# ruc-aimc-lab/GeoFormer

Hardware: AMD Instinct MI355X
Metric: image-pairs/sec (640x640) (higher is better)
Workload: dtype f16

## Files before the change

### geoformer_amd/csrc/k9_encoder_fused.hip

```cpp
#include <math.h>

#include <type_traits>

#include "gf_common.h"
#include "k9_args.h"

#ifndef K9P_TRACE
#define K9P_TRACE 0
#endif
#ifndef K9P_ABLATE
#define K9P_ABLATE 0
#endif
#if K9P_TRACE
__device__ long long k9p_trace[1024 * 8 * 24];
#define K9P_T(slot) do { if (lane == 0 && blockIdx.x < 1024) k9p_trace[(blockIdx.x * 8 + wave) * 24 + (slot)] = (long long)__builtin_amdgcn_s_memtime(); } while (0)
extern "C" int gf_debug_k9p_trace(long long* out) {
    return (int)hipMemcpyFromSymbol(out, HIP_SYMBOL(k9p_trace), sizeof(long long) * 1024 * 8 * 24);
}
#else
#define K9P_T(slot)
#endif

namespace {

constexpr int C = 256, D = 32, NH = 8;
constexpr int TM = 128;
constexpr int FRAG = 1024, BLK = 16 * FRAG;
constexpr int X_OFF = 0;
constexpr int W_OFF = 65536;
constexpr int E_OFF = W_OFF + 3 * BLK;
constexpr int VEC_OFF = E_OFF + 32768;
constexpr int KS_OFF = VEC_OFF + 4 * C * 4;
constexpr int ST_OFF = KS_OFF + 512;
constexpr int LDS_BYTES = ST_OFF + 8 * 64 * 8;
constexpr int NB_Q = 8, NB_M = 8, NB_SLICE = 12, NB_KV = 16;

using EncArgs = GfEncArgs;

template <typename T>
__device__ __forceinline__ typename Mma32<T>::Frag pack8(float a0, float a1, float a2, float a3, float a4, float a5, float a6,
                                                          float a7) {
    typedef T t2 __attribute__((ext_vector_type(2)));
    typedef float f2 __attribute__((ext_vector_type(2)));
    const t2 p0 = __builtin_convertvector(f2{a0, a1}, t2), p1 = __builtin_convertvector(f2{a2, a3}, t2);
    const t2 p2 = __builtin_convertvector(f2{a4, a5}, t2), p3 = __builtin_convertvector(f2{a6, a7}, t2);
    return typename Mma32<T>::Frag{p0[0], p0[1], p1[0], p1[1], p2[0], p2[1], p3[0], p3[1]};
}
template <typename T>
__device__ __forceinline__ typename Mma32<T>::Frag pack_step(const v16f& a, int s) {
    return s == 0 ? pack8<T>(a[0], a[1], a[2], a[3], a[4], a[5], a[6], a[7])
                  : pack8<T>(a[8], a[9], a[10], a[11], a[12], a[13], a[14], a[15]);
}
template <typename F>
__device__ __forceinline__ F relu_packed(const F& f) {
    typedef short v8s __attribute__((ext_vector_type(8)));
    const v8s x = __builtin_bit_cast(v8s, f);
    return __builtin_bit_cast(F, x & ~(x >> 15));
}
__device__ __forceinline__ float phi(float x) {
    return fmaxf(x, 0.f) + __builtin_amdgcn_fmed3f(__builtin_amdgcn_exp2f(x * 1.44269504088896341f), 0.f, 1.f);
}
__device__ __forceinline__ v16f zero16() { return v16f{0.f, 0.f, 0.f, 0.f, 0.f, 0.f, 0.f, 0.f, 0.f, 0.f, 0.f, 0.f, 0.f, 0.f, 0.f, 0.f}; }
__device__ __forceinline__ int fresh_lane() {
    int l;
    asm volatile("v_mbcnt_lo_u32_b32 %0, -1, 0\n\tv_mbcnt_hi_u32_b32 %0, -1, %0" : "=v"(l));
    return l;
}
__device__ __forceinline__ float half_sum(float x) {
    const gf_v2u sw = __builtin_amdgcn_permlane32_swap(__float_as_uint(x), __float_as_uint(x), false, false);
    return __uint_as_float(sw.x) + __uint_as_float(sw.y);
}
__device__ __forceinline__ float dot8(const v8h& a, const v8h& b, float c) {
    typedef _Float16 h2 __attribute__((ext_vector_type(2)));
#pragma unroll
    for (int i = 0; i < 4; ++i) c = __builtin_amdgcn_fdot2(h2{a[2 * i], a[2 * i + 1]}, h2{b[2 * i], b[2 * i + 1]}, c, false);
    return c;
}
__device__ __forceinline__ float dot8(const v8b& a, const v8b& b, float c) {
    typedef __bf16 b2 __attribute__((ext_vector_type(2)));
#pragma unroll
    for (int i = 0; i < 4; ++i) c = __builtin_amdgcn_fdot2_f32_bf16(b2{a[2 * i], a[2 * i + 1]}, b2{b[2 * i], b[2 * i + 1]}, c, false);
    return c;
}

template <typename T>
struct PMma {
    static __device__ __forceinline__ void mma(const typename Mma32<T>::Frag& a, const typename Mma32<T>::Frag& b, v16f& c) {
#if K9P_ABLATE == 4
        asm volatile("" : "+v"(c) : "v"(a), "v"(b));
#else
        Mma32<T>::mma(a, b, c);
#endif
    }
};

struct Ring {
    __amdgpu_buffer_rsrc_t rs;
    __amdgpu_buffer_rsrc_t rs2;
    char* smem;
    int voff;
    int wave;
    int rbase;
    int blk, nblk;
};
__device__ __forceinline__ Ring ring_make(const void* wstream, char* smem, int wave, int lane, int nblk, const void* wstream2, int nblk2) {
    return Ring{__builtin_amdgcn_make_buffer_rsrc(const_cast<void*>(wstream), 0, nblk * BLK, 0x00020000),
                __builtin_amdgcn_make_buffer_rsrc(const_cast<void*>(wstream2 ? wstream2 : wstream), 0, wstream2 ? nblk2 * BLK : 0, 0x00020000),
                smem, lane * 16 + wave * 2 * FRAG, wave, W_OFF + (wave & 1) * 8 * FRAG + lane * 16, 0, nblk};
}
__device__ __forceinline__ void dma_piece(const Ring& g, int slot, int b, int i) {
#if K9P_ABLATE == 1
    if (b >= 3) return;
#endif
    const bool second = b >= g.nblk;
    __builtin_amdgcn_raw_ptr_buffer_load_lds(second ? g.rs2 : g.rs,
                                             (__attribute__((address_space(3))) void*)(g.smem + W_OFF + slot * BLK + (g.wave * 2 + i) * FRAG), 16,
                                             g.voff, (second ? b - g.nblk : b) * BLK + i * FRAG, 0, 0);
}
template <int VM>
__device__ __forceinline__ void turn() {
    asm volatile("s_waitcnt vmcnt(%0) lgkmcnt(0)" ::"n"(VM) : "memory");
#if K9P_ABLATE != 2
    __builtin_amdgcn_s_barrier();
#endif
}
__device__ __forceinline__ void xbar() {
    asm volatile("s_waitcnt lgkmcnt(0)" ::: "memory");
    __builtin_amdgcn_s_barrier();
}
template <typename Frag>
__device__ __forceinline__ Frag lds_frag(const char* p) { return *reinterpret_cast<const Frag*>(p); }
template <typename Frag>
__device__ __forceinline__ Frag ring_frag(const char* p) {
#if K9P_ABLATE == 3
    Frag f; asm volatile("" : "=v"(f)); return f;
#else
    return *reinterpret_cast<const Frag*>(p);
#endif
}

#define K9_GAP(DMA, READS, VALU)                                            \
    __builtin_amdgcn_sched_group_barrier(0x008, 1, 0);                      \
    if (DMA) __builtin_amdgcn_sched_group_barrier(0x010, 1, 0);             \
    if (READS) __builtin_amdgcn_sched_group_barrier(0x100, READS, 0);       \
    if (VALU) __builtin_amdgcn_sched_group_barrier(0x002, VALU, 0);
template <int NX0, int NX4, int VM, int NV0 = 0, int NV4 = 0, typename Frag, typename MF, typename H0, typename H4>
__device__ __forceinline__ void pblock(Ring& g, Frag (&F)[8], int slot, MF mma, H0 h0, H4 h4) {
    const char* pc = g.smem + g.rbase + slot * BLK;
    mma(0);
    F[6] = ring_frag<Frag>(pc + 6 * FRAG);
    h0();
    mma(1);
    F[7] = ring_frag<Frag>(pc + 7 * FRAG);
    mma(2);
    mma(3);
    K9_GAP(false, 1 + NX0, NV0) K9_GAP(false, 1, NV0) K9_GAP(false, 0, NV0) K9_GAP(false, 0, NV0)
    __builtin_amdgcn_sched_barrier(0);
    turn<VM>();
    const char* p = g.smem + g.rbase + ((slot + 1) % 3) * BLK;
    mma(4);
    dma_piece(g, slot, g.blk + 3, 0);
    F[0] = ring_frag<Frag>(p);
    F[1] = ring_frag<Frag>(p + FRAG);
    h4();
    mma(5);
    dma_piece(g, slot, g.blk + 3, 1);
    F[2] = ring_frag<Frag>(p + 2 * FRAG);
    F[3] = ring_frag<Frag>(p + 3 * FRAG);
    mma(6);
    F[4] = ring_frag<Frag>(p + 4 * FRAG);
    mma(7);
    F[5] = ring_frag<Frag>(p + 5 * FRAG);
    K9_GAP(true, 2 + NX4, NV4) K9_GAP(true, 2, NV4) K9_GAP(false, 1, NV4) K9_GAP(false, 1, NV4)
    __builtin_amdgcn_sched_barrier(0);
    ++g.blk;
}
#undef K9_GAP
__device__ __forceinline__ void ring_start(const Ring& g) {
#pragma unroll
    for (int b = 0; b < 3; ++b) {
        dma_piece(g, b, b, 0);
        dma_piece(g, b, b, 1);
    }
    __builtin_amdgcn_sched_barrier(0);
}
template <typename Frag>
__device__ __forceinline__ void load_block0(const Ring& g, Frag (&f)[8]) {
    const char* p = g.smem + g.rbase;
#pragma unroll
    for (int i = 0; i < 6; ++i) f[i] = ring_frag<Frag>(p + i * FRAG);
}

template <typename T>
__device__ __forceinline__ void tile_dma(const T* base, long ld, int rows_total, int row0, int nrows, char* smem, int off, int wave, int lane,
                                         int waves) {
    const __amdgpu_buffer_rsrc_t rs = __builtin_amdgcn_make_buffer_rsrc(const_cast<T*>(base), 0, 0x7FFFFFFF, 0x00020000);
    const int planes_pieces = nrows / 8;
    const int total = 4 * planes_pieces, per = total / waves;
#pragma unroll
    for (int i = 0; i < 8; ++i) {
        if (i < per) {
            const int q = wave * per + i, kc = q / planes_pieces, rp = q - kc * planes_pieces;
            const int row = rp * 8 + (lane >> 3), c = (lane & 7) ^ ((row >> 1) & 7);
            const int r = min(row0 + row, rows_total - 1);
            __builtin_amdgcn_raw_ptr_buffer_load_lds(rs, (__attribute__((address_space(3))) void*)(smem + off + kc * (nrows * 128) + rp * 1024), 16,
                                                     (int)(r * ld * 2) + kc * 128 + c * 16, 0, 0, 0);
        }
    }
}

template <typename T>
__device__ __forceinline__ void kv_tail(Ring& ring, typename Mma32<T>::Frag (&F)[8], char* smem, unsigned valid,
                                        float* dst, int wave, int lane, int tid, int slot0);

template <typename T, int ACT, bool ATTN>
__global__ __launch_bounds__(512) void enc_layer(EncArgs a) {
    using Mm = Mma32<T>;
    using Frag = typename Mm::Frag;
    extern __shared__ __attribute__((aligned(16))) char smem[];
    const int tid = threadIdx.x, lane = tid & 63, wave = __builtin_amdgcn_readfirstlane(tid >> 6), h2 = lane >> 5, lr = lane & 31;
    const int w = wave & 1, grp = wave >> 1;
    const int n = blockIdx.x / a.tiles, tile = blockIdx.x - n * a.tiles;
    const int t0 = tile * TM;
    const T* xg = (const T*)a.x + (size_t)n * a.L * a.ldx;
    constexpr int NBLK = (ATTN ? NB_Q : 0) + NB_M + 4 * NB_SLICE;
    float* vec = reinterpret_cast<float*>(smem + VEC_OFF);
    const bool tail = ATTN && a.wstream_tail != nullptr && n >= a.tail_first;
    K9P_T(0);
    Ring ring = ring_make(a.wstream, smem, wave, lane, NBLK, tail ? a.wstream_tail : nullptr, NB_KV);
    const int mytok = t0 + grp * 32 + lr;
    const int myrow = grp * 32 + lr;
    const float lnv0 = a.ln[tid], lnv1 = a.ln[512 + tid];
    unsigned char qm = 1;
    if (a.q_mask != nullptr) qm = a.q_mask[(size_t)n * a.L + min(mytok, a.L - 1)];
    float kvv[2][8], ksv = 0.f;
    if constexpr (ATTN) {
        const float* kvf = a.kvfinal + (size_t)n * (C * D + C);
#pragma unroll
        for (int p = 0; p < 2; ++p) {
            const int sl = p * 512 + tid, ln = sl & 63, hs = sl >> 6, hh = hs >> 1, s = hs & 1;
            const float* src = kvf + (size_t)(hh * D + 16 * s + 4 * (ln >> 5)) * D + (ln & 31);
#pragma unroll
            for (int j = 0; j < 8; ++j) kvv[p][j] = src[((j >> 2) * 8 + (j & 3)) * D];
        }
        {
            const int tq = tid & 255, j = tq & 7, hx = (tq >> 3) & 1, sx = (tq >> 4) & 1, hh = tq >> 5;
            ksv = kvf[C * D + hh * D + 16 * sx + 8 * (j >> 2) + 4 * hx + (j & 3)];
        }
    }
    __builtin_amdgcn_sched_barrier(0);
    tile_dma<T>(xg, a.ldx, a.L, t0, TM, smem, X_OFF, wave, lane, 8);
    dma_piece(ring, 0, 0, 0);
    dma_piece(ring, 0, 0, 1);
    __builtin_amdgcn_sched_barrier(0);
    K9P_T(13);
    vec[tid] = lnv0;
    vec[512 + tid] = lnv1;
    const float qmul = qm != 0 ? 1.f : 0.f;
    if constexpr (ATTN) {
        const float inv_s = 1.0f / (float)a.S;
#pragma unroll
        for (int p = 0; p < 2; ++p) {
            const int sl = p * 512 + tid, ln = sl & 63, hs = sl >> 6;
            *reinterpret_cast<Frag*>(smem + E_OFF + hs * FRAG + ln * 16) =
                pack8<T>(kvv[p][0] * inv_s, kvv[p][1] * inv_s, kvv[p][2] * inv_s, kvv[p][3] * inv_s, kvv[p][4] * inv_s, kvv[p][5] * inv_s,
                         kvv[p][6] * inv_s, kvv[p][7] * inv_s);
        }
        reinterpret_cast<T*>(smem + KS_OFF)[tid & 255] = gf_from_float<T>(ksv * inv_s);
    }
    Frag ma[16];
    if constexpr (!ATTN) {
        const T* mg = (const T*)a.msg + (size_t)n * a.L * a.ldm;
#pragma unroll
        for (int half = 0; half < 2; ++half) {
            tile_dma<T>(mg, a.ldm, a.L, t0 + half * 64, 64, smem, E_OFF, wave, lane, 8);
            asm volatile("s_waitcnt vmcnt(0)" ::: "memory");
            __builtin_amdgcn_s_barrier();
            if ((grp >> 1) == half) {
                const int row = (grp & 1) * 32 + lr;
#pragma unroll
                for (int t = 0; t < 8; ++t)
#pragma unroll
                    for (int s = 0; s < 2; ++s) {
                        const int c0 = 32 * t + 16 * s + 4 * h2, ch = c0 >> 3;
                        const char* p0 = smem + E_OFF + (ch >> 3) * 8192 + gf_lds_off(row, ch & 7) + (c0 & 7) * 2;
                        const char* p1 = smem + E_OFF + ((ch + 1) >> 3) * 8192 + gf_lds_off(row, (ch + 1) & 7) + (c0 & 7) * 2;
                        typedef short v4s __attribute__((ext_vector_type(4)));
                        typedef short v8s __attribute__((ext_vector_type(8)));
                        const v4s lo = *reinterpret_cast<const v4s*>(p0), hi = *reinterpret_cast<const v4s*>(p1);
                        const v8s both = __builtin_shufflevector(lo, hi, 0, 1, 2, 3, 4, 5, 6, 7);
                        ma[2 * t + s] = __builtin_bit_cast(Frag, both);
                    }
            }
            xbar();
        }
    }
    K9P_T(14);
    asm volatile("s_waitcnt vmcnt(0) lgkmcnt(0)" ::: "memory");
    K9P_T(15);
    __builtin_amdgcn_s_barrier();
    dma_piece(ring, 1, 1, 0);
    dma_piece(ring, 1, 1, 1);
    dma_piece(ring, 2, 2, 0);
    dma_piece(ring, 2, 2, 1);
    __builtin_amdgcn_sched_barrier(0);

    K9P_T(1);
    Frag F[8];
    load_block0(ring, F);
    auto xfrag = [&](int ks) { return lds_frag<Frag>(smem + X_OFF + (ks >> 2) * 16384 + gf_lds_off(myrow, 2 * (ks & 3) + h2)); };
    char* const ex = smem + E_OFF + grp * 8192 + lane * 16;
    auto ex_put = [&](int i, const Frag& f) { *reinterpret_cast<Frag*>(ex + (4 * w + i) * FRAG) = f; };
    auto ex_get = [&](int s) { return lds_frag<Frag>(ex + s * FRAG); };
    int slot = 0;

    Frag kvf[4][2];
    v16f qacc[2];
    v16f num;
    float den = 0.f;
    Frag p0, p1, msg0, msg1;
    const float eps_s = ATTN ? a.attn_eps / (float)a.S : 0.f;
    auto att_a0 = [&](int t) {
        const int hh = 4 * w + t;
        const Frag ks0 = lds_frag<Frag>(smem + KS_OFF + ((hh * 2 + 0) * 2 + h2) * 16);
        const v16f& qh = qacc[t & 1];
        p0 = pack8<T>(phi(qh[0]), phi(qh[1]), phi(qh[2]), phi(qh[3]), phi(qh[4]), phi(qh[5]), phi(qh[6]), phi(qh[7]));
        den = dot8(p0, ks0, 0.f);
    };
    auto att_a1 = [&](int t) {
        const int hh = 4 * w + t;
        const Frag ks1 = lds_frag<Frag>(smem + KS_OFF + ((hh * 2 + 1) * 2 + h2) * 16);
        const v16f& qh = qacc[t & 1];
        p1 = pack8<T>(phi(qh[8]), phi(qh[9]), phi(qh[10]), phi(qh[11]), phi(qh[12]), phi(qh[13]), phi(qh[14]), phi(qh[15]));
        den = dot8(p1, ks1, den);
        num = zero16();
        Mm::mma(kvf[t][0], p0, num);
        Mm::mma(kvf[t][1], p1, num);
    };
    auto att_b0 = [&] {
        const float z = __builtin_amdgcn_rcpf(half_sum(den) + eps_s) * qmul;
#pragma unroll
        for (int r = 0; r < 16; ++r) num[r] *= z;
        msg0 = pack_step<T>(num, 0);
        msg1 = pack_step<T>(num, 1);
    };
    auto att_put = [&](int t) {
        *reinterpret_cast<Frag*>(ex + (4 * w + 2 * (t & 1)) * FRAG) = msg0;
        *reinterpret_cast<Frag*>(ex + (4 * w + 2 * (t & 1) + 1) * FRAG) = msg1;
    };
    auto att_get = [&](int t) {
        ma[2 * t] = ex_get(2 * (t & 1));
        ma[2 * t + 1] = ex_get(2 * (t & 1) + 1);
        ma[8 + 2 * t] = ex_get(4 + 2 * (t & 1));
        ma[9 + 2 * t] = ex_get(5 + 2 * (t & 1));
    };
    if constexpr (ATTN) {
#pragma unroll
// ... 170 lines not shown
        hn[1] = zero16();
        auto w1xn = [&](int j) { PMma<T>::mma(F[j], X[j >> 1], hn[j & 1]); };
#pragma unroll
        for (int b = 0; b < 4; ++b) {
            if (b < 3) pblock<2, 2, 2>(ring, F, slot, w1xn, [&] { xh0(b); }, [&] { xh4(b); });
            else pblock<2, 1, 2>(ring, F, slot, w1xn, [&] { xh0(b); }, [&] { H[0] = ex_get(0); });
            slot = (slot + 1) % 3;
        }
#pragma unroll
        for (int b = 0; b < 4; ++b) {
            pblock<1, 1, 2>(ring, F, slot, [&](int j) { PMma<T>::mma(F[j], H[j >> 2], o[j & 3]); }, [&] { H[1] = ex_get(2 * b + 1); },
                            [&] { if (b < 3) H[0] = ex_get(2 * b + 2); });
            slot = (slot + 1) % 3;
        }
#pragma unroll
        for (int b = 0; b < 4; ++b) {
            auto mm = [&](int j) { PMma<T>::mma(F[j], ma[4 * b + (j >> 1)], hn[j & 1]); };
            if (b < 3) pblock<0, 0, 2>(ring, F, slot, mm, [] {}, [] {});
            else pblock<0, 2, 2>(ring, F, slot, mm, [] {}, [&] { X[0] = xfrag(0); X[1] = xfrag(1); });
            slot = (slot + 1) % 3;
        }
        hd[0] = hn[0];
        hd[1] = hn[1];
        act_put();
    }
    K9P_T(8);
    {
        xbar();
        int slot = STAGE_SLOT;
        H[0] = ex_get(0);
#pragma unroll
        for (int b = 0; b < 4; ++b) {
            pblock<1, 1, 2>(ring, F, slot, [&](int j) { PMma<T>::mma(F[j], H[j >> 2], o[j & 3]); }, [&] { H[1] = ex_get(2 * b + 1); },
                            [&] { if (b < 3) H[0] = ex_get(2 * b + 2); });
            slot = (slot + 1) % 3;
        }
    }
    K9P_T(10);

    float mean2, rstd2;
    {
        float s2 = 0.f, q2 = 0.f;
#pragma unroll
        for (int t = 0; t < 4; ++t) stats_add(o[t], s2, q2);
        s2 = half_sum(s2);
        q2 = half_sum(q2);
        stats_put(s2, q2);
        xbar();
        stats_finish(s2, q2, a.eps2, mean2, rstd2);
    }
    const float nmr2 = -mean2 * rstd2;
    K9P_T(11);
    const bool keep = a.flag == nullptr || __builtin_amdgcn_readfirstlane(a.flag[((size_t)n * a.L + t0) / a.flag_rows]) != 0;
    {
        typedef T v4t __attribute__((ext_vector_type(4)));
        if (keep) {
            int xs[8];
#pragma unroll
            for (int k = 0; k < 8; ++k) xs[k] = X_OFF + w * 32768 + gf_lds_off(myrow, k) + h2 * 8;
            struct FinOps { v4t x[4]; LnOps ln[2]; };
            auto fin_ops = [&](int t) {
                FinOps fo;
#pragma unroll
                for (int g = 0; g < 4; ++g) fo.x[g] = *reinterpret_cast<const v4t*>(smem + xs[4 * (t & 1) + g] + (t >> 1) * 16384);
                fo.ln[0] = ln_ops(vec + 2 * C, vec + 3 * C, 4 * w + t, 0);
                fo.ln[1] = ln_ops(vec + 2 * C, vec + 3 * C, 4 * w + t, 1);
                return fo;
            };
            FinOps fo[2];
            fo[0] = fin_ops(0);
#pragma unroll
            for (int t = 0; t < 4; ++t) {
                if (t < 3) fo[(t + 1) & 1] = fin_ops(t + 1);
                const FinOps& p = fo[t & 1];
#pragma unroll
                for (int g = 0; g < 4; ++g) {
                    const v4f y = ln_apply(o[t], g, p.ln[g >> 1].ga[g & 1], p.ln[g >> 1].be[g & 1], nmr2, rstd2);
                    v4t ov;
                    ov[0] = gf_from_float<T>(gf_to_float(p.x[g][0]) + y.x);
                    ov[1] = gf_from_float<T>(gf_to_float(p.x[g][1]) + y.y);
                    ov[2] = gf_from_float<T>(gf_to_float(p.x[g][2]) + y.z);
                    ov[3] = gf_from_float<T>(gf_to_float(p.x[g][3]) + y.w);
                    *reinterpret_cast<v4t*>(smem + xs[4 * (t & 1) + g] + (t >> 1) * 16384) = ov;
                }
            }
            __builtin_amdgcn_fence(__ATOMIC_RELEASE, "wavefront");
            __builtin_amdgcn_wave_barrier();
            __builtin_amdgcn_fence(__ATOMIC_ACQUIRE, "wavefront");
        }
        K9P_T(17);
        T* og = (T*)a.out + (size_t)n * a.L * a.ldo;
        const __amdgpu_buffer_rsrc_t ors = __builtin_amdgcn_make_buffer_rsrc(og, 0, (int)min((long)a.L * a.ldo * 2, 0x7FFFFFFFL), 0x00020000);
        const int c16 = lane & 15, rsel = lane >> 4;
        v4u rows[8];
#pragma unroll
        for (int it = 0; it < 8; ++it)
            rows[it] = *reinterpret_cast<const v4u*>(smem + X_OFF + (2 * w + (c16 >> 3)) * 16384 + gf_lds_off(grp * 32 + 4 * it + rsel, c16 & 7));
#pragma unroll
        for (int it = 0; it < 8; ++it) {
            const int tg = t0 + grp * 32 + 4 * it + rsel;
            __builtin_amdgcn_raw_buffer_store_b128(rows[it], ors, (int)(tg * a.ldo * 2) + (16 * w + c16) * 16, 0, 0);
        }
    }
    K9P_T(12);
    if constexpr (ATTN) {
        if (tail) {
            xbar();
            const int tl = fresh_lane();
            const int ttok = t0 + grp * 32 + (tl & 31);
            const bool ok = ttok < a.L && (a.q_mask == nullptr || a.q_mask[(size_t)n * a.L + min(ttok, a.L - 1)] != 0);
            const unsigned valid = (unsigned)__ballot(ok && (tl >> 5) == 0);
            kv_tail<T>(ring, F, smem, valid, a.part + ((size_t)(n - a.tail_first) * a.tiles + tile) * (C * D + C), wave, tl, wave * 64 + tl, NBLK % 3);
        }
    }
}

template <typename T>
__device__ __forceinline__ void kv_tail(Ring& ring, typename Mma32<T>::Frag (&F)[8], char* smem, unsigned valid,
                                        float* dst, int wave, int lane, int tid, int slot0) {
    using Mm = Mma32<T>;
    using Frag = typename Mm::Frag;
    const int h2 = lane >> 5, lr = lane & 31, w = wave & 1, grp = wave >> 1;
    const int myrow = grp * 32 + lr;
    auto xfrag = [&](int ks) { return lds_frag<Frag>(smem + X_OFF + (ks >> 2) * 16384 + gf_lds_off(myrow, 2 * (ks & 3) + h2)); };
    int slot = slot0;
    auto project = [&](v16f (&acc)[4], auto between) {
#pragma unroll
        for (int t = 0; t < 4; ++t) acc[t] = zero16();
        Frag X[2];
        X[0] = xfrag(0);
#pragma unroll
        for (int b = 0; b < 8; ++b) {
            pblock<1, 1, 2>(ring, F, slot, [&](int j) { PMma<T>::mma(X[j >> 2], F[j], acc[j & 3]); }, [&] { X[1] = xfrag(2 * b + 1); },
                            [&] { X[0] = xfrag(b < 7 ? 2 * b + 2 : 15); between(b); });
            slot = (slot + 1) % 3;
        }
    };
    Frag kf[4][2];
    float ksum[4];
    float vm[16];
#pragma unroll
    for (int r = 0; r < 16; ++r) vm[r] = ((valid >> gf_acc_row(r, h2)) & 1u) ? 1.f : 0.f;
    v16f k[4];
    project(k, [](int) {});
    float srun = 0.f;
    auto phi_half = [&](int st) {
        const int hh = st >> 1, sx = st & 1;
        float s = sx == 0 ? 0.f : srun;
#pragma unroll
        for (int r = 8 * sx; r < 8 * sx + 8; ++r) {
            const float p = phi(k[hh][r]) * vm[r];
            k[hh][r] = p;
            s += p;
        }
        kf[hh][sx] = pack_step<T>(k[hh], sx);
        if (sx == 0) srun = s;
        else ksum[hh] = half_sum(s);
    };
    v16f kv[4];
    {
        v16f v[4];
        project(v, phi_half);
#pragma unroll
        for (int hh = 0; hh < 4; ++hh) {
            kv[hh] = zero16();
            Mm::mma(kf[hh][0], pack_step<T>(v[hh], 0), kv[hh]);
            Mm::mma(kf[hh][1], pack_step<T>(v[hh], 1), kv[hh]);
        }
    }
    constexpr int KVN = 4 * 16 * 64, SLOT = KVN + 4 * 64;
    float* red = reinterpret_cast<float*>(smem);
    asm volatile("s_waitcnt vmcnt(0)" ::: "memory");
    __syncthreads();
#pragma unroll
    for (int hh = 0; hh < 4; ++hh) {
#pragma unroll
        for (int r = 0; r < 16; ++r) red[wave * SLOT + (hh * 16 + r) * 64 + lane] = kv[hh][r];
        red[wave * SLOT + KVN + hh * 64 + lane] = ksum[hh];
    }
    __syncthreads();
#pragma unroll 4
    for (int e2 = tid; e2 < 2 * KVN; e2 += 512) {
        const int wh = e2 >> 12, e = e2 & (KVN - 1);
        const float* r0 = red + wh * SLOT + e;
        const float sum = (r0[0] + r0[4 * SLOT]) + (r0[2 * SLOT] + r0[6 * SLOT]);
        const int hh = 4 * wh + (e >> 10), r = (e >> 6) & 15, ln = e & 63;
        dst[(size_t)(hh * D + gf_acc_row(r, ln >> 5)) * D + (ln & 31)] = sum;
    }
    if (tid < 256) {
        const int wh = tid >> 7, e = tid & 127, hh = e >> 5, ln = e & 31;
        const float* r0 = red + wh * SLOT + KVN + hh * 64 + ln;
        dst[C * D + (4 * wh + hh) * D + ln] = (r0[0] + r0[4 * SLOT]) + (r0[2 * SLOT] + r0[6 * SLOT]);
    }
}

template <typename T>
__global__ __launch_bounds__(512) void enc_kv_state(EncArgs a) {
    using Mm = Mma32<T>;
    using Frag = typename Mm::Frag;
    extern __shared__ __attribute__((aligned(16))) char smem[];
    const int tid = threadIdx.x, lane = tid & 63, wave = __builtin_amdgcn_readfirstlane(tid >> 6), h2 = lane >> 5, lr = lane & 31;
    const int n = blockIdx.x / a.tiles, tile = blockIdx.x - n * a.tiles;
    const int t0 = tile * TM;
    const T* xg = (const T*)a.x + (size_t)n * a.S * a.ldx;
    Ring ring = ring_make(a.wstream, smem, wave, lane, NB_KV, nullptr, 0);
    tile_dma<T>(xg, a.ldx, a.S, t0, TM, smem, X_OFF, wave, lane, 8);
    dma_piece(ring, 0, 0, 0);
    dma_piece(ring, 0, 0, 1);
    __builtin_amdgcn_sched_barrier(0);
    const int mytok = t0 + (wave >> 1) * 32 + lr;
    const bool ok = mytok < a.S && (a.kv_mask == nullptr || a.kv_mask[(size_t)n * a.S + min(mytok, a.S - 1)] != 0);
    const unsigned valid = (unsigned)__ballot(ok && h2 == 0);
    dma_piece(ring, 1, 1, 0);
    dma_piece(ring, 1, 1, 1);
    dma_piece(ring, 2, 2, 0);
    dma_piece(ring, 2, 2, 1);
    __builtin_amdgcn_sched_barrier(0);
    asm volatile("s_waitcnt vmcnt(4) lgkmcnt(0)" ::: "memory");
    __builtin_amdgcn_s_barrier();
    Frag F[8];
    load_block0(ring, F);
    kv_tail<T>(ring, F, smem, valid, a.part + ((size_t)n * a.tiles + tile) * (C * D + C), wave, lane, tid, 0);
}

__global__ void enc_kv_reduce(const float* part, float* fin, int tiles, int len) {
    const int n = blockIdx.y, i = blockIdx.x * blockDim.x + threadIdx.x;
    if (i >= len) return;
    const float* p = part + (size_t)n * tiles * len + i;
    float s = 0.f;
    int c = 0;
    for (; c + 10 <= tiles; c += 10) {
        float v[10];
#pragma unroll
        for (int j = 0; j < 10; ++j) v[j] = p[(size_t)(c + j) * len];
#pragma unroll
        for (int j = 0; j < 10; ++j) s += v[j];
    }
    for (; c < tiles; ++c) s += p[(size_t)c * len];
    fin[(size_t)n * len + i] = s;
}

template <typename T>
void pair_launch(const EncArgs& a, int act, bool attn, hipStream_t st) {
    const dim3 grid(a.N * a.tiles);
    if (attn) {
        if (act == 0) enc_layer<T, 0, true><<<grid, 512, LDS_BYTES, st>>>(a);
        else enc_layer<T, 1, true><<<grid, 512, LDS_BYTES, st>>>(a);
    } else {
        if (act == 0) enc_layer<T, 0, false><<<grid, 512, LDS_BYTES, st>>>(a);
        else enc_layer<T, 1, false><<<grid, 512, LDS_BYTES, st>>>(a);
    }
}

std::atomic<uint64_t> pair_attr_done{0};
template <typename K>
void pair_allow_lds(K kern) { (void)hipFuncSetAttribute((const void*)kern, hipFuncAttributeMaxDynamicSharedMemorySize, LDS_BYTES); }
void pair_init() {
    if (!gf_first_use_on_device(pair_attr_done)) return;
    pair_allow_lds(enc_layer<_Float16, 0, true>); pair_allow_lds(enc_layer<_Float16, 1, true>);
    pair_allow_lds(enc_layer<_Float16, 0, false>); pair_allow_lds(enc_layer<_Float16, 1, false>);
    pair_allow_lds(enc_kv_state<_Float16>);
    pair_allow_lds(enc_layer<gf_bf16, 0, true>); pair_allow_lds(enc_layer<gf_bf16, 1, true>);
    pair_allow_lds(enc_layer<gf_bf16, 0, false>); pair_allow_lds(enc_layer<gf_bf16, 1, false>);
    pair_allow_lds(enc_kv_state<gf_bf16>);
}

}

extern "C" size_t gf_encoder_kv_workspace_bytes(int N, int S) {
    if (N <= 0 || S <= 0) return 0;
    const size_t tiles = (S + TM - 1) / TM, len = (size_t)C * D + C;
    return gf_align_up(sizeof(float) * N * tiles * len, 256);
}

extern "C" int gf_encoder_kv_state(const void* src, long ld, int dtype, int N, int S, const uint8_t* kv_mask,
                                   const void* wstream_kv, float* kv_state, void* workspace, size_t workspace_bytes,
                                   void* stream) {
    GF_CHECK_ARG(src && wstream_kv && kv_state, "null pointer");
    GF_CHECK_ARG(N > 0 && S > 0, "empty problem");
    GF_CHECK_ARG(dtype == GF_F16 || dtype == GF_BF16, "the fused encoder kernels are built for 16-bit storage (GF_F16 / GF_BF16)");
    GF_CHECK_ARG((ld * 2) % 16 == 0 && (uintptr_t)src % 16 == 0 && (uintptr_t)wstream_kv % 16 == 0, "operands must be 16-byte aligned");
    if (workspace == nullptr || workspace_bytes < gf_encoder_kv_workspace_bytes(N, S)) {
        gf_set_error("gf_encoder_kv_state: workspace too small");
        return GF_ERR_WORKSPACE;
    }
    pair_init();
    EncArgs a{};
    a.x = src; a.ldx = ld; a.N = N; a.L = S; a.S = S; a.tiles = (S + TM - 1) / TM; a.kv_mask = kv_mask; a.wstream = wstream_kv;
    a.part = (float*)workspace;
    hipStream_t st = (hipStream_t)stream;
    const int len = C * D + C;
    void* pt = gf_prof_begin("enc_kv_state", st, 2.0 * N * (double)S * C * (2.0 * C + 2.0 * D));
    if (dtype == GF_F16) enc_kv_state<_Float16><<<N * a.tiles, 512, LDS_BYTES, st>>>(a);
    else enc_kv_state<gf_bf16><<<N * a.tiles, 512, LDS_BYTES, st>>>(a);
    enc_kv_reduce<<<dim3((len + 255) / 256, N), 256, 0, st>>>(a.part, kv_state, a.tiles, len);
    gf_prof_end("enc_kv_state", pt, st);
    GF_CHECK_LAUNCH();
    return GF_OK;
}

extern "C" int gf_encoder_layer_kv(const void* x, long ldx, const float* kv_state, int S, const uint8_t* q_mask, float attn_eps,
                                   const void* wstream, const float* ln_params, float eps1, float eps2, int activation, void* out,
                                   long ldo, int dtype, int N, int L, const void* wstream_tail, int tail_first, float* kv_state_out,
                                   void* workspace, size_t workspace_bytes, void* stream) {
    GF_CHECK_ARG(x && wstream && ln_params && out && kv_state, "null pointer");
    GF_CHECK_ARG(wstream_tail && kv_state_out && tail_first >= 0 && tail_first < N, "the state tail needs its weight stream, its output and 0 <= tail_first < N");
    GF_CHECK_ARG(N > 0 && L > 0 && S > 0, "empty problem");
    GF_CHECK_ARG(dtype == GF_F16 || dtype == GF_BF16, "the fused encoder kernels are built for 16-bit storage (GF_F16 / GF_BF16)");
    GF_CHECK_ARG(activation == 0 || activation == 1, "activation: 0 = ReLU, 1 = Tanh");
    GF_CHECK_ARG((ldx * 2) % 16 == 0 && (ldo * 2) % 16 == 0, "rows must be 16-byte aligned");
    GF_CHECK_ARG((uintptr_t)x % 16 == 0 && (uintptr_t)out % 16 == 0 && (uintptr_t)wstream % 16 == 0 && (uintptr_t)wstream_tail % 16 == 0,
                 "tensors must be 16-byte aligned");
    const int nt = N - tail_first;
    if (workspace == nullptr || workspace_bytes < gf_encoder_kv_workspace_bytes(nt, L)) {
        gf_set_error("gf_encoder_layer_kv: workspace too small");
        return GF_ERR_WORKSPACE;
    }
    pair_init();
    EncArgs a{};
    a.x = x; a.ldx = ldx; a.kvfinal = kv_state; a.q_mask = q_mask; a.wstream = wstream; a.ln = ln_params;
    a.eps1 = eps1; a.eps2 = eps2; a.attn_eps = attn_eps; a.out = out; a.ldo = ldo; a.N = N; a.L = L; a.S = S;
    a.tiles = (L + TM - 1) / TM;
    a.wstream_tail = wstream_tail; a.tail_first = tail_first; a.part = (float*)workspace;
    hipStream_t st = (hipStream_t)stream;
    const double per_tok = 2.0 * C * C + 2.0 * C * (D + 1) + 2.0 * C * C + 8.0 * C * C + 4.0 * C * C;
    const double tail_tok = 2.0 * C * (2.0 * C + 2.0 * D);
    void* pt = gf_prof_begin("enc_layer", st, per_tok * N * (double)L + tail_tok * nt * (double)L);
    const int len = C * D + C;
    if (dtype == GF_F16) pair_launch<_Float16>(a, activation, true, st);
    else pair_launch<gf_bf16>(a, activation, true, st);
    enc_kv_reduce<<<dim3((len + 255) / 256, nt), 256, 0, st>>>(a.part, kv_state_out, a.tiles, len);
    gf_prof_end("enc_layer", pt, st);
    GF_CHECK_LAUNCH();
    return GF_OK;
}

extern "C" int gf_encoder_layer(const void* x, long ldx, const void* msg, long ldm, const float* kv_state, int S,
                                const uint8_t* q_mask, float attn_eps, const void* wstream, const float* ln_params, float eps1,
                                float eps2, int activation, const int32_t* row_flag, int flag_rows, void* out, long ldo, int dtype,
                                int N, int L, void* stream) {
    GF_CHECK_ARG(x && wstream && ln_params && out, "null pointer");
    GF_CHECK_ARG((msg != nullptr) != (kv_state != nullptr), "exactly one of msg (attention output) and kv_state (linear attention) is given");
    GF_CHECK_ARG(N > 0 && L > 0 && (kv_state == nullptr || S > 0), "empty problem");
    GF_CHECK_ARG(dtype == GF_F16 || dtype == GF_BF16, "the fused encoder kernels are built for 16-bit storage (GF_F16 / GF_BF16)");
    GF_CHECK_ARG(activation == 0 || activation == 1, "activation: 0 = ReLU, 1 = Tanh");
    GF_CHECK_ARG((ldx * 2) % 16 == 0 && (ldo * 2) % 16 == 0 && (msg == nullptr || (ldm * 2) % 16 == 0), "rows must be 16-byte aligned");
    GF_CHECK_ARG((uintptr_t)x % 16 == 0 && (uintptr_t)out % 16 == 0 && (uintptr_t)msg % 16 == 0 && (uintptr_t)wstream % 16 == 0,
                 "tensors must be 16-byte aligned");
    GF_CHECK_ARG(row_flag == nullptr || flag_rows > 0, "flag_rows must be > 0");
    pair_init();
    EncArgs a{};
    a.x = x; a.ldx = ldx; a.msg = msg; a.ldm = ldm; a.kvfinal = kv_state; a.q_mask = q_mask; a.wstream = wstream; a.ln = ln_params;
    a.eps1 = eps1; a.eps2 = eps2; a.attn_eps = attn_eps; a.out = out; a.ldo = ldo; a.N = N; a.L = L; a.S = S > 0 ? S : 1;
    a.tiles = (L + TM - 1) / TM; a.flag = row_flag; a.flag_rows = flag_rows;
    hipStream_t st = (hipStream_t)stream;
    const bool attn = kv_state != nullptr;
    const double per_tok = (attn ? 2.0 * C * C + 2.0 * C * (D + 1) : 0.0) + 2.0 * C * C + 8.0 * C * C + 4.0 * C * C;
    void* pt = gf_prof_begin("enc_layer", st, per_tok * N * (double)L);
    if (dtype == GF_F16) pair_launch<_Float16>(a, activation, attn, st);
    else pair_launch<gf_bf16>(a, activation, attn, st);
    gf_prof_end("enc_layer", pt, st);
    GF_CHECK_LAUNCH();
    return GF_OK;
}
```

Measured before the change: 730.5.

## Make encoder layer kernel persistent and prefetch next tile during epilogue

```diff
diff --git a/geoformer_amd/csrc/k9_encoder_fused.hip b/geoformer_amd/csrc/k9_encoder_fused.hip
--- a/geoformer_amd/csrc/k9_encoder_fused.hip
+++ b/geoformer_amd/csrc/k9_encoder_fused.hip
@@ -13,12 +13,14 @@
 #endif
 #if K9P_TRACE
 __device__ long long k9p_trace[1024 * 8 * 24];
-#define K9P_T(slot) do { if (lane == 0 && blockIdx.x < 1024) k9p_trace[(blockIdx.x * 8 + wave) * 24 + (slot)] = (long long)__builtin_amdgcn_s_memtime(); } while (0)
+#define K9P_TI(slot, tile_it) do { if (lane == 0 && walk_it == (tile_it) && blockIdx.x < 1024) k9p_trace[(blockIdx.x * 8 + wave) * 24 + (slot)] = (long long)__builtin_amdgcn_s_memtime(); } while (0)
+#define K9P_T(slot) K9P_TI(slot, 1)
 extern "C" int gf_debug_k9p_trace(long long* out) {
     return (int)hipMemcpyFromSymbol(out, HIP_SYMBOL(k9p_trace), sizeof(long long) * 1024 * 8 * 24);
 }
 #else
 #define K9P_T(slot)
+#define K9P_TI(slot, tile_it)
 #endif
 
 namespace {
@@ -34,6 +36,7 @@
 constexpr int ST_OFF = KS_OFF + 512;
 constexpr int LDS_BYTES = ST_OFF + 8 * 64 * 8;
 constexpr int NB_Q = 8, NB_M = 8, NB_SLICE = 12, NB_KV = 16;
+constexpr int NST_ROWS = 8, NST_PART = 16;
 
 using EncArgs = GfEncArgs;
 
@@ -102,11 +105,15 @@
     int wave;
     int rbase;
     int blk, nblk;
+    bool wrap;
+    int hold;
 };
-__device__ __forceinline__ Ring ring_make(const void* wstream, char* smem, int wave, int lane, int nblk, const void* wstream2, int nblk2) {
+__device__ __forceinline__ Ring ring_make(const void* wstream, char* smem, int wave, int lane, int nblk, const void* wstream2, int nblk2,
+                                          bool wrap = false) {
     return Ring{__builtin_amdgcn_make_buffer_rsrc(const_cast<void*>(wstream), 0, nblk * BLK, 0x00020000),
-                __builtin_amdgcn_make_buffer_rsrc(const_cast<void*>(wstream2 ? wstream2 : wstream), 0, wstream2 ? nblk2 * BLK : 0, 0x00020000),
-                smem, lane * 16 + wave * 2 * FRAG, wave, W_OFF + (wave & 1) * 8 * FRAG + lane * 16, 0, nblk};
+                __builtin_amdgcn_make_buffer_rsrc(const_cast<void*>(wstream2 ? wstream2 : wstream), 0, wstream2 ? nblk2 * BLK : wrap ? 3 * BLK : 0,
+                                                  0x00020000),
+                smem, lane * 16 + wave * 2 * FRAG, wave, W_OFF + (wave & 1) * 8 * FRAG + lane * 16, 0, nblk, wrap, 0};
 }
 __device__ __forceinline__ void dma_piece(const Ring& g, int slot, int b, int i) {
 #if K9P_ABLATE == 1
@@ -115,11 +122,17 @@
     const bool second = b >= g.nblk;
     __builtin_amdgcn_raw_ptr_buffer_load_lds(second ? g.rs2 : g.rs,
                                              (__attribute__((address_space(3))) void*)(g.smem + W_OFF + slot * BLK + (g.wave * 2 + i) * FRAG), 16,
-                                             g.voff, (second ? b - g.nblk : b) * BLK + i * FRAG, 0, 0);
+                                             g.voff, (second ? (g.wrap ? slot : b - g.nblk) : b) * BLK + i * FRAG, 0, 0);
+}
+__device__ __forceinline__ void wait_vm(int nst) {
+    if (nst == 0) asm volatile("s_waitcnt vmcnt(0) lgkmcnt(0)" ::: "memory");
+    else if (nst == NST_ROWS) asm volatile("s_waitcnt vmcnt(%0) lgkmcnt(0)" ::"n"(NST_ROWS) : "memory");
+    else asm volatile("s_waitcnt vmcnt(%0) lgkmcnt(0)" ::"n"(NST_PART) : "memory");
 }
 template <int VM>
-__device__ __forceinline__ void turn() {
-    asm volatile("s_waitcnt vmcnt(%0) lgkmcnt(0)" ::"n"(VM) : "memory");
+__device__ __forceinline__ void turn(int hold) {
+    if (hold == 0) asm volatile("s_waitcnt vmcnt(%0) lgkmcnt(0)" ::"n"(VM) : "memory");
+    else wait_vm(hold);
 #if K9P_ABLATE != 2
     __builtin_amdgcn_s_barrier();
 #endif
@@ -156,7 +169,8 @@
     mma(3);
     K9_GAP(false, 1 + NX0, NV0) K9_GAP(false, 1, NV0) K9_GAP(false, 0, NV0) K9_GAP(false, 0, NV0)
     __builtin_amdgcn_sched_barrier(0);
-    turn<VM>();
+    turn<VM>(g.hold);
+    g.hold = 0;
     const char* p = g.smem + g.rbase + ((slot + 1) % 3) * BLK;
     mma(4);
     dma_piece(g, slot, g.blk + 3, 0);
@@ -210,52 +224,102 @@
 }
 
 template <typename T>
+__device__ __forceinline__ void tile_dma_own(const T* base, long ld, int rows_total, int row0, char* smem, int wave, int lane, int first = 0,
+                                             int count = 8) {
+    const __amdgpu_buffer_rsrc_t rs = __builtin_amdgcn_make_buffer_rsrc(const_cast<T*>(base), 0, 0x7FFFFFFF, 0x00020000);
+#pragma unroll
+    for (int i = first; i < first + count; ++i) {
+        const int kc = 2 * (wave & 1) + (i >> 2), rp = (wave >> 1) * 4 + (i & 3);
+        const int row = rp * 8 + (lane >> 3), c = (lane & 7) ^ ((row >> 1) & 7);
+        const int r = min(row0 + row, rows_total - 1);
+        __builtin_amdgcn_raw_ptr_buffer_load_lds(rs, (__attribute__((address_space(3))) void*)(smem + X_OFF + kc * (TM * 128) + rp * 1024), 16,
+                                                 (int)(r * ld * 2) + kc * 128 + c * 16, 0, 0, 0);
+    }
+}
+
+template <typename T, bool WALK, typename Between>
 __device__ __forceinline__ void kv_tail(Ring& ring, typename Mma32<T>::Frag (&F)[8], char* smem, unsigned valid,
-                                        float* dst, int wave, int lane, int tid, int slot0);
+                                        float* dst, int wave, int lane, int tid, int slot0, Between between);
 
 template <typename T, int ACT, bool ATTN>
 __global__ __launch_bounds__(512) void enc_layer(EncArgs a) {
     using Mm = Mma32<T>;
     using Frag = typename Mm::Frag;
     extern __shared__ __attribute__((aligned(16))) char smem[];
-    const int tid = threadIdx.x, lane = tid & 63, wave = __builtin_amdgcn_readfirstlane(tid >> 6), h2 = lane >> 5, lr = lane & 31;
+    const int wave = __builtin_amdgcn_readfirstlane(threadIdx.x >> 6);
     const int w = wave & 1, grp = wave >> 1;
-    const int n = blockIdx.x / a.tiles, tile = blockIdx.x - n * a.tiles;
-    const int t0 = tile * TM;
-    const T* xg = (const T*)a.x + (size_t)n * a.L * a.ldx;
     constexpr int NBLK = (ATTN ? NB_Q : 0) + NB_M + 4 * NB_SLICE;
     float* vec = reinterpret_cast<float*>(smem + VEC_OFF);
+    const int total = a.N * a.tiles, G = gridDim.x;
+    unsigned char qm = 1;
+    float kvv[2][8], ksv = 0.f;
+    auto req_image = [&](int idx2) {
+        const int l2 = fresh_lane(), tid2 = wave * 64 + l2;
+        const int n2 = idx2 / a.tiles, t02 = (idx2 - n2 * a.tiles) * TM;
+        {
+            const bool masked = a.q_mask != nullptr;
+            const unsigned char* qsrc = masked ? a.q_mask + (size_t)n2 * a.L : reinterpret_cast<const unsigned char*>(a.ln);
+            const unsigned char v = qsrc[masked ? min(t02 + grp * 32 + (l2 & 31), a.L - 1) : 0];
+            qm = masked ? v : (unsigned char)1;
+        }
+        if constexpr (ATTN) {
+            const float* kvf = a.kvfinal + (size_t)n2 * (C * D + C);
+#pragma unroll
+            for (int p = 0; p < 2; ++p) {
+                const int sl = p * 512 + tid2, ln = sl & 63, hs = sl >> 6, hh = hs >> 1, s = hs & 1;
+                const float* src = kvf + (size_t)(hh * D + 16 * s + 4 * (ln >> 5)) * D + (ln & 31);
+#pragma unroll
+                for (int j = 0; j < 8; ++j) kvv[p][j] = src[((j >> 2) * 8 + (j & 3)) * D];
+            }
+            {
+                const int tq = tid2 & 255, j = tq & 7, hx = (tq >> 3) & 1, sx = (tq >> 4) & 1, hh = tq >> 5;
+                ksv = kvf[C * D + hh * D + 16 * sx + 8 * (j >> 2) + 4 * hx + (j & 3)];
+            }
+        }
+        __builtin_amdgcn_sched_barrier(0);
+    };
+    auto req_tile = [&](int idx2, int first, int count) {
+        const int n2 = idx2 / a.tiles, t02 = (idx2 - n2 * a.tiles) * TM;
+        tile_dma_own<T>((const T*)a.x + (size_t)n2 * a.L * a.ldx, a.ldx, a.L, t02, smem, wave, fresh_lane(), first, count);
+        __builtin_amdgcn_sched_barrier(0);
+    };
+    auto req_rest = [&](int idx2, const Ring& rg, int nring) {
+        const int n2 = idx2 / a.tiles, t02 = (idx2 - n2 * a.tiles) * TM;
+        if constexpr (!ATTN) tile_dma<T>((const T*)a.msg + (size_t)n2 * a.L * a.ldm, a.ldm, a.L, t02, 64, smem, E_OFF, wave, fresh_lane(), 8);
+#pragma unroll
+        for (int b = 0; b < 3; ++b)
+            if (b < nring) {
+                dma_piece(rg, b, b, 0);
+                dma_piece(rg, b, b, 1);
+            }
+        __builtin_amdgcn_sched_barrier(0);
+    };
+    auto request = [&](int idx2, const Ring& rg, int nring) {
+        req_image(idx2);
+        req_tile(idx2, 0, 8);
+        req_rest(idx2, rg, nring);
+    };
+    {
+        const int tid = threadIdx.x;
+        const float lnv0 = a.ln[tid], lnv1 = a.ln[512 + tid];
+        request(blockIdx.x, ring_make(a.wstream, smem, wave, tid & 63, NBLK, nullptr, 0), 1);
+        vec[tid] = lnv0;
+        vec[512 + tid] = lnv1;
+    }
+    int nst = 0;
+#pragma unroll 1
+    for (int idx = blockIdx.x, walk_it = 0; idx < total; idx += G, ++walk_it) {
+    const int lane = fresh_lane(), tid = wave * 64 + lane, h2 = lane >> 5, lr = lane & 31;
+    const int n = idx / a.tiles, tile = idx - n * a.tiles;
+    const int t0 = tile * TM;
     const bool tail = ATTN && a.wstream_tail != nullptr && n >= a.tail_first;
+    const bool has_next = idx + G < total;
+    K9P_TI(19, 2);
     K9P_T(0);
-    Ring ring = ring_make(a.wstream, smem, wave, lane, NBLK, tail ? a.wstream_tail : nullptr, NB_KV);
-    const int mytok = t0 + grp * 32 + lr;
+    Ring ring = ring_make(a.wstream, smem, wave, lane, NBLK, tail ? a.wstream_tail : nullptr, NB_KV, !tail && has_next);
+    ring.hold = nst;
     const int myrow = grp * 32 + lr;
-    const float lnv0 = a.ln[tid], lnv1 = a.ln[512 + tid];
-    unsigned char qm = 1;
-    if (a.q_mask != nullptr) qm = a.q_mask[(size_t)n * a.L + min(mytok, a.L - 1)];
-    float kvv[2][8], ksv = 0.f;
-    if constexpr (ATTN) {
-        const float* kvf = a.kvfinal + (size_t)n * (C * D + C);
-#pragma unroll
-        for (int p = 0; p < 2; ++p) {
-            const int sl = p * 512 + tid, ln = sl & 63, hs = sl >> 6, hh = hs >> 1, s = hs & 1;
-            const float* src = kvf + (size_t)(hh * D + 16 * s + 4 * (ln >> 5)) * D + (ln & 31);
-#pragma unroll
-            for (int j = 0; j < 8; ++j) kvv[p][j] = src[((j >> 2) * 8 + (j & 3)) * D];
-        }
-        {
-            const int tq = tid & 255, j = tq & 7, hx = (tq >> 3) & 1, sx = (tq >> 4) & 1, hh = tq >> 5;
-            ksv = kvf[C * D + hh * D + 16 * sx + 8 * (j >> 2) + 4 * hx + (j & 3)];
-        }
-    }
-    __builtin_amdgcn_sched_barrier(0);
-    tile_dma<T>(xg, a.ldx, a.L, t0, TM, smem, X_OFF, wave, lane, 8);
-    dma_piece(ring, 0, 0, 0);
-    dma_piece(ring, 0, 0, 1);
-    __builtin_amdgcn_sched_barrier(0);
     K9P_T(13);
-    vec[tid] = lnv0;
-    vec[512 + tid] = lnv1;
     const float qmul = qm != 0 ? 1.f : 0.f;
     if constexpr (ATTN) {
         const float inv_s = 1.0f / (float)a.S;
@@ -273,8 +337,12 @@
         const T* mg = (const T*)a.msg + (size_t)n * a.L * a.ldm;
 #pragma unroll
         for (int half = 0; half < 2; ++half) {
-            tile_dma<T>(mg, a.ldm, a.L, t0 + half * 64, 64, smem, E_OFF, wave, lane, 8);
-            asm volatile("s_waitcnt vmcnt(0)" ::: "memory");
+            if (half == 0) {
+                wait_vm(nst);
+            } else {
+                tile_dma<T>(mg, a.ldm, a.L, t0 + half * 64, 64, smem, E_OFF, wave, lane, 8);
+                asm volatile("s_waitcnt vmcnt(0)" ::: "memory");
+            }
             __builtin_amdgcn_s_barrier();
             if ((grp >> 1) == half) {
                 const int row = (grp & 1) * 32 + lr;
@@ -296,13 +364,15 @@
         }
     }
     K9P_T(14);
-    asm volatile("s_waitcnt vmcnt(0) lgkmcnt(0)" ::: "memory");
+    wait_vm(nst);
     K9P_T(15);
     __builtin_amdgcn_s_barrier();
-    dma_piece(ring, 1, 1, 0);
-    dma_piece(ring, 1, 1, 1);
-    dma_piece(ring, 2, 2, 0);
-    dma_piece(ring, 2, 2, 1);
+    if (walk_it == 0) {
+        dma_piece(ring, 1, 1, 0);
+        dma_piece(ring, 1, 1, 1);
+        dma_piece(ring, 2, 2, 0);
+        dma_piece(ring, 2, 2, 1);
+    }
     __builtin_amdgcn_sched_barrier(0);
 
     K9P_T(1);
@@ -579,8 +649,24 @@
     const float nmr2 = -mean2 * rstd2;
     K9P_T(11);
     const bool keep = a.flag == nullptr || __builtin_amdgcn_readfirstlane(a.flag[((size_t)n * a.L + t0) / a.flag_rows]) != 0;
+    const bool ahead = has_next && !tail;
+    if (ahead) req_image(idx + G);
     {
         typedef T v4t __attribute__((ext_vector_type(4)));
+        const int c8 = lane & 7, r8 = lane >> 3;
+        v4u rows[2][4];
+        auto plane_out = [&](int p) {
+            __builtin_amdgcn_fence(__ATOMIC_RELEASE, "wavefront");
+            __builtin_amdgcn_wave_barrier();
+            __builtin_amdgcn_fence(__ATOMIC_ACQUIRE, "wavefront");
+#pragma unroll
+            for (int i = 0; i < 4; ++i)
+                rows[p][i] = *reinterpret_cast<const v4u*>(smem + X_OFF + (2 * w + p) * 16384 + gf_lds_off(grp * 32 + 8 * i + r8, c8));
+            if (ahead) {
+                asm volatile("s_waitcnt lgkmcnt(0)" ::: "memory");
+                req_tile(idx + G, 4 * p, 4);
+            }
+        };
         if (keep) {
             int xs[8];
 #pragma unroll
@@ -610,24 +696,27 @@
                     ov[3] = gf_from_float<T>(gf_to_float(p.x[g][3]) + y.w);
                     *reinterpret_cast<v4t*>(smem + xs[4 * (t & 1) + g] + (t >> 1) * 16384) = ov;
                 }
+                if (t & 1) plane_out(t >> 1);
             }
-            __builtin_amdgcn_fence(__ATOMIC_RELEASE, "wavefront");
-            __builtin_amdgcn_wave_barrier();
-            __builtin_amdgcn_fence(__ATOMIC_ACQUIRE, "wavefront");
+        } else {
+            plane_out(0);
+            plane_out(1);
         }
         K9P_T(17);
+        if (ahead) {
+            req_rest(idx + G, ring, 0);
+            K9P_T(18);
+        }
         T* og = (T*)a.out + (size_t)n * a.L * a.ldo;
         const __amdgpu_buffer_rsrc_t ors = __builtin_amdgcn_make_buffer_rsrc(og, 0, (int)min((long)a.L * a.ldo * 2, 0x7FFFFFFFL), 0x00020000);
-        const int c16 = lane & 15, rsel = lane >> 4;
-        v4u rows[8];
-#pragma unroll
-        for (int it = 0; it < 8; ++it)
-            rows[it] = *reinterpret_cast<const v4u*>(smem + X_OFF + (2 * w + (c16 >> 3)) * 16384 + gf_lds_off(grp * 32 + 4 * it + rsel, c16 & 7));
-#pragma unroll
-        for (int it = 0; it < 8; ++it) {
-            const int tg = t0 + grp * 32 + 4 * it + rsel;
-            __builtin_amdgcn_raw_buffer_store_b128(rows[it], ors, (int)(tg * a.ldo * 2) + (16 * w + c16) * 16, 0, 0);
-        }
+#pragma unroll
+        for (int p = 0; p < 2; ++p)
+#pragma unroll
+            for (int i = 0; i < 4; ++i) {
+                const int tg = t0 + grp * 32 + 8 * i + r8;
+                __builtin_amdgcn_raw_buffer_store_b128(rows[p][i], ors, (int)(tg * a.ldo * 2) + (2 * w + p) * 128 + c8 * 16, 0, 0);
+            }
+        nst = NST_ROWS;
     }
     K9P_T(12);
     if constexpr (ATTN) {
@@ -637,14 +726,17 @@
             const int ttok = t0 + grp * 32 + (tl & 31);
             const bool ok = ttok < a.L && (a.q_mask == nullptr || a.q_mask[(size_t)n * a.L + min(ttok, a.L - 1)] != 0);
             const unsigned valid = (unsigned)__ballot(ok && (tl >> 5) == 0);
-            kv_tail<T>(ring, F, smem, valid, a.part + ((size_t)(n - a.tail_first) * a.tiles + tile) * (C * D + C), wave, tl, wave * 64 + tl, NBLK % 3);
-        }
-    }
-}
-
-template <typename T>
+            kv_tail<T, true>(ring, F, smem, valid, a.part + ((size_t)(n - a.tail_first) * a.tiles + tile) * (C * D + C), wave, tl, wave * 64 + tl, NBLK % 3,
+                       [&] { if (has_next) request(idx + G, ring, 3); });
+            nst = NST_PART;
+        }
+    }
+    }
+}
+
+template <typename T, bool WALK, typename Between>
 __device__ __forceinline__ void kv_tail(Ring& ring, typename Mma32<T>::Frag (&F)[8], char* smem, unsigned valid,
-                                        float* dst, int wave, int lane, int tid, int slot0) {
+                                        float* dst, int wave, int lane, int tid, int slot0, Between between) {
     using Mm = Mma32<T>;
     using Frag = typename Mm::Frag;
     const int h2 = lane >> 5, lr = lane & 31, w = wave & 1, grp = wave >> 1;
@@ -696,6 +788,7 @@
         }
     }
     constexpr int KVN = 4 * 16 * 64, SLOT = KVN + 4 * 64;
+    static_assert(8 * SLOT * 4 <= VEC_OFF, "the LayerNorm parameters of a walking workgroup stay parked");
     float* red = reinterpret_cast<float*>(smem);
     asm volatile("s_waitcnt vmcnt(0)" ::: "memory");
     __syncthreads();
@@ -706,18 +799,46 @@
         red[wave * SLOT + KVN + hh * 64 + lane] = ksum[hh];
     }
     __syncthreads();
+    if constexpr (!WALK) {
 #pragma unroll 4
-    for (int e2 = tid; e2 < 2 * KVN; e2 += 512) {
-        const int wh = e2 >> 12, e = e2 & (KVN - 1);
-        const float* r0 = red + wh * SLOT + e;
-        const float sum = (r0[0] + r0[4 * SLOT]) + (r0[2 * SLOT] + r0[6 * SLOT]);
-        const int hh = 4 * wh + (e >> 10), r = (e >> 6) & 15, ln = e & 63;
-        dst[(size_t)(hh * D + gf_acc_row(r, ln >> 5)) * D + (ln & 31)] = sum;
-    }
-    if (tid < 256) {
-        const int wh = tid >> 7, e = tid & 127, hh = e >> 5, ln = e & 31;
-        const float* r0 = red + wh * SLOT + KVN + hh * 64 + ln;
-        dst[C * D + (4 * wh + hh) * D + ln] = (r0[0] + r0[4 * SLOT]) + (r0[2 * SLOT] + r0[6 * SLOT]);
+        for (int e2 = tid; e2 < 2 * KVN; e2 += 512) {
+            const int wh = e2 >> 12, e = e2 & (KVN - 1);
+            const float* r0 = red + wh * SLOT + e;
+            const float sum = (r0[0] + r0[4 * SLOT]) + (r0[2 * SLOT] + r0[6 * SLOT]);
+            const int hh = 4 * wh + (e >> 10), r = (e >> 6) & 15, ln = e & 63;
+            dst[(size_t)(hh * D + gf_acc_row(r, ln >> 5)) * D + (ln & 31)] = sum;
+        }
+        if (tid < 256) {
+            const int wh = tid >> 7, e = tid & 127, hh = e >> 5, ln = e & 31;
+            const float* r0 = red + wh * SLOT + KVN + hh * 64 + ln;
+            dst[C * D + (4 * wh + hh) * D + ln] = (r0[0] + r0[4 * SLOT]) + (r0[2 * SLOT] + r0[6 * SLOT]);
+        }
+    } else {
+        static_assert(2 * KVN / 512 == NST_PART, "stores of a partial per lane");
+        float sums[NST_PART], kss = 0.f;
+#pragma unroll
+        for (int i = 0; i < NST_PART; ++i) {
+            const int e2 = tid + 512 * i, wh = e2 >> 12, e = e2 & (KVN - 1);
+            const float* r0 = red + wh * SLOT + e;
+            sums[i] = (r0[0] + r0[4 * SLOT]) + (r0[2 * SLOT] + r0[6 * SLOT]);
+        }
+        if (tid < 256) {
+            const int wh = tid >> 7, e = tid & 127, hh = e >> 5, ln = e & 31;
+            const float* r0 = red + wh * SLOT + KVN + hh * 64 + ln;
+            kss = (r0[0] + r0[4 * SLOT]) + (r0[2 * SLOT] + r0[6 * SLOT]);
+        }
+        xbar();
+        between();
+#pragma unroll
+        for (int i = 0; i < NST_PART; ++i) {
+            const int e2 = tid + 512 * i, wh = e2 >> 12, e = e2 & (KVN - 1);
+            const int hh = 4 * wh + (e >> 10), r = (e >> 6) & 15, ln = e & 63;
+            dst[(size_t)(hh * D + gf_acc_row(r, ln >> 5)) * D + (ln & 31)] = sums[i];
+        }
+        if (tid < 256) {
+            const int wh = tid >> 7, e = tid & 127, hh = e >> 5, ln = e & 31;
+            dst[C * D + (4 * wh + hh) * D + ln] = kss;
+        }
     }
 }
 
@@ -747,7 +868,7 @@
     __builtin_amdgcn_s_barrier();
     Frag F[8];
     load_block0(ring, F);
-    kv_tail<T>(ring, F, smem, valid, a.part + ((size_t)n * a.tiles + tile) * (C * D + C), wave, lane, tid, 0);
+    kv_tail<T, false>(ring, F, smem, valid, a.part + ((size_t)n * a.tiles + tile) * (C * D + C), wave, lane, tid, 0, [] {});
 }
 
 __global__ void enc_kv_reduce(const float* part, float* fin, int tiles, int len) {
@@ -767,9 +888,14 @@
     fin[(size_t)n * len + i] = s;
 }
 
+int pair_grid(const EncArgs& a, int cus) {
+    const long nt = (long)a.N * a.tiles;
+    return (int)(nt < cus ? nt : cus);
+}
+
 template <typename T>
-void pair_launch(const EncArgs& a, int act, bool attn, hipStream_t st) {
-    const dim3 grid(a.N * a.tiles);
+void pair_launch(const EncArgs& a, int act, bool attn, int cus, hipStream_t st) {
+    const dim3 grid(pair_grid(a, cus));
     if (attn) {
         if (act == 0) enc_layer<T, 0, true><<<grid, 512, LDS_BYTES, st>>>(a);
         else enc_layer<T, 1, true><<<grid, 512, LDS_BYTES, st>>>(a);
@@ -780,16 +906,29 @@
 }
 
 std::atomic<uint64_t> pair_attr_done{0};
+std::atomic<int> pair_cus[64];
 template <typename K>
 void pair_allow_lds(K kern) { (void)hipFuncSetAttribute((const void*)kern, hipFuncAttributeMaxDynamicSharedMemorySize, LDS_BYTES); }
-void pair_init() {
-    if (!gf_first_use_on_device(pair_attr_done)) return;
+int pair_cu_count() {
+    int dev = 0;
+    const bool known = hipGetDevice(&dev) == hipSuccess && dev >= 0 && dev < 64;
+    int cus = known ? pair_cus[dev].load(std::memory_order_relaxed) : 0;
+    if (cus <= 0) {
+        if (hipDeviceGetAttribute(&cus, hipDeviceAttributeMultiprocessorCount, known ? dev : 0) != hipSuccess || cus <= 0) cus = 256;
+        if (known) pair_cus[dev].store(cus, std::memory_order_relaxed);
+    }
+    return cus;
+}
+int pair_init() {
+    const int cus = pair_cu_count();
+    if (!gf_first_use_on_device(pair_attr_done)) return cus;
     pair_allow_lds(enc_layer<_Float16, 0, true>); pair_allow_lds(enc_layer<_Float16, 1, true>);
     pair_allow_lds(enc_layer<_Float16, 0, false>); pair_allow_lds(enc_layer<_Float16, 1, false>);
     pair_allow_lds(enc_kv_state<_Float16>);
     pair_allow_lds(enc_layer<gf_bf16, 0, true>); pair_allow_lds(enc_layer<gf_bf16, 1, true>);
     pair_allow_lds(enc_layer<gf_bf16, 0, false>); pair_allow_lds(enc_layer<gf_bf16, 1, false>);
     pair_allow_lds(enc_kv_state<gf_bf16>);
+    return cus;
 }
 
 }
@@ -811,7 +950,7 @@
         gf_set_error("gf_encoder_kv_state: workspace too small");
         return GF_ERR_WORKSPACE;
     }
-    pair_init();
+    (void)pair_init();
     EncArgs a{};
     a.x = src; a.ldx = ld; a.N = N; a.L = S; a.S = S; a.tiles = (S + TM - 1) / TM; a.kv_mask = kv_mask; a.wstream = wstream_kv;
     a.part = (float*)workspace;
@@ -843,7 +982,7 @@
         gf_set_error("gf_encoder_layer_kv: workspace too small");
         return GF_ERR_WORKSPACE;
     }
-    pair_init();
+    const int cus = pair_init();
     EncArgs a{};
     a.x = x; a.ldx = ldx; a.kvfinal = kv_state; a.q_mask = q_mask; a.wstream = wstream; a.ln = ln_params;
     a.eps1 = eps1; a.eps2 = eps2; a.attn_eps = attn_eps; a.out = out; a.ldo = ldo; a.N = N; a.L = L; a.S = S;
@@ -854,8 +993,8 @@
     const double tail_tok = 2.0 * C * (2.0 * C + 2.0 * D);
     void* pt = gf_prof_begin("enc_layer", st, per_tok * N * (double)L + tail_tok * nt * (double)L);
     const int len = C * D + C;
-    if (dtype == GF_F16) pair_launch<_Float16>(a, activation, true, st);
-    else pair_launch<gf_bf16>(a, activation, true, st);
+    if (dtype == GF_F16) pair_launch<_Float16>(a, activation, true, cus, st);
+    else pair_launch<gf_bf16>(a, activation, true, cus, st);
     enc_kv_reduce<<<dim3((len + 255) / 256, nt), 256, 0, st>>>(a.part, kv_state_out, a.tiles, len);
     gf_prof_end("enc_layer", pt, st);
     GF_CHECK_LAUNCH();
@@ -875,7 +1014,7 @@
     GF_CHECK_ARG((uintptr_t)x % 16 == 0 && (uintptr_t)out % 16 == 0 && (uintptr_t)msg % 16 == 0 && (uintptr_t)wstream % 16 == 0,
                  "tensors must be 16-byte aligned");
     GF_CHECK_ARG(row_flag == nullptr || flag_rows > 0, "flag_rows must be > 0");
-    pair_init();
+    const int cus = pair_init();
     EncArgs a{};
     a.x = x; a.ldx = ldx; a.msg = msg; a.ldm = ldm; a.kvfinal = kv_state; a.q_mask = q_mask; a.wstream = wstream; a.ln = ln_params;
     a.eps1 = eps1; a.eps2 = eps2; a.attn_eps = attn_eps; a.out = out; a.ldo = ldo; a.N = N; a.L = L; a.S = S > 0 ? S : 1;
@@ -884,8 +1023,8 @@
     const bool attn = kv_state != nullptr;
     const double per_tok = (attn ? 2.0 * C * C + 2.0 * C * (D + 1) : 0.0) + 2.0 * C * C + 8.0 * C * C + 4.0 * C * C;
     void* pt = gf_prof_begin("enc_layer", st, per_tok * N * (double)L);
-    if (dtype == GF_F16) pair_launch<_Float16>(a, activation, attn, st);
-    else pair_launch<gf_bf16>(a, activation, attn, st);
+    if (dtype == GF_F16) pair_launch<_Float16>(a, activation, attn, cus, st);
+    else pair_launch<gf_bf16>(a, activation, attn, cus, st);
     gf_prof_end("enc_layer", pt, st);
     GF_CHECK_LAUNCH();
     return GF_OK;
```

Result: no change. 732.6 (median of 4 runs) (+0.3%).
